# google-research/simclr

Measured on AMD Instinct MI355X. Metric: images/sec (whole node), ResNet-50 1x SimCLR pretraining step @224px, higher is better.
Workload: dtype f32; 1 GPU; ResNet-50 1x, 224x224, 2 views/image, per-GPU batch 512, global batch 512, NT-Xent T=0.1 + linear-eval head + LARS, global BN, dp1; global_batch=512, parallelism=dp1

## Files before the change

### simclr_amd/csrc/conv.hip

```cpp
#include "common.h"
#include <stdlib.h>
#include <string.h>
#include <mutex>
#include <type_traits>

namespace {

enum { MODE_FWD = 0, MODE_DGRAD = 1 };

struct ConvP {
  const void* x;
  const void* w;
  void* y;
  float* stats;
  int V, IH, IW, IC, OH, OW, N, KH, KW, stride, pad;
  int pixpitch;
  int M, K;
  int nslot, accumulate;
  int m_tiles, n_tiles;
  int cs, py, px, cls_h, cls_w;
  int ntaps;
  int taps[9];
  unsigned long long tap_w, dy_w, dx_w;
  const void* bn_x;
// ... 2158 lines not shown
      const int row = q >> 3, j = (q >> 2) & 1, gq = q & 3;
      u32x4* w0 = (u32x4*)(xs + off_of(row, (j * 8 + gq) * 16));
      u32x4* w1 = (u32x4*)(xs + off_of(row, (j * 8 + 4 + gq) * 16));
      u32x4 hi, lo;
      split_terms2(*w0, *w1, hi, lo);
      *w0 = hi; *w1 = lo;
    }
  };

  auto compute = [&](int s) __attribute__((always_inline)) {
    const unsigned char* xs = smem + s * stage_bytes;
    const unsigned char* ds = xs + p.hpp * RB;
    u32x4 dh[4], dl[4];
#pragma unroll
    for (int ni = 0; ni < 4; ++ni) {
      const int o0 = b_lo[ni] & ~7, o1 = hi_of(b_lo[ni]);
      dh[ni] = frag(ds, o0, o1);
      dl[ni] = frag(ds, o0 ^ 64, o1 ^ 64);
    }
    const int jw = p.W - gx;
    const unsigned lowm = jw >= 8 ? 0xffu : ((1u << jw) - 1u);
    const int y1 = (gy + 1 == p.H) ? 0 : gy + 1;
    const unsigned up = (gy > 0 ? lowm : 0u) | (y1 > 0 ? (0xffu & ~lowm) : 0u);
    const unsigned dn = (gy < p.H - 1 ? lowm : 0u) | (y1 < p.H - 1 ? (0xffu & ~lowm) : 0u);
    const unsigned lf = 0xffu & ~((gx == 0 ? 1u : 0u) | (jw < 8 ? (1u << jw) : 0u));
    const unsigned rt = 0xffu & ~((jw - 1 < 8 ? (1u << (jw - 1)) : 0u) | (jw - 1 + p.W < 8 ? (1u << (jw - 1 + p.W)) : 0u));
    __builtin_amdgcn_s_setprio(1);
#pragma unroll
    for (int t = 0; t < 9; ++t) {
      const int ty = t / 3, tx = t % 3;
      const int o0 = a_lo[t] & ~7, o1 = hi_of(a_lo[t]);
      u32x4 xh = frag(xs, o0, o1);
      u32x4 xl = frag(xs, o0 ^ 64, o1 ^ 64);
      if (t != 4) {
        const unsigned m8 = (ty == 0 ? up : ty == 2 ? dn : 0xffu) & (tx == 0 ? lf : tx == 2 ? rt : 0xffu);
#pragma unroll
        for (int d = 0; d < 4; ++d) {
          const unsigned w = ((unsigned)__builtin_amdgcn_sbfe((int)m8, 2 * d, 1) & 0x0000ffffu) |
                             ((unsigned)__builtin_amdgcn_sbfe((int)m8, 2 * d + 1, 1) & 0xffff0000u);
          xh[d] &= w; xl[d] &= w;
        }
      }
#pragma unroll
      for (int ni = 0; ni < 4; ++ni) acc[t][ni] = mma_bf16(dl[ni], xh, acc[t][ni]);
#pragma unroll
      for (int ni = 0; ni < 4; ++ni) acc[t][ni] = mma_bf16(dh[ni], xl, acc[t][ni]);
#pragma unroll
      for (int ni = 0; ni < 4; ++ni) acc[t][ni] = mma_bf16(dh[ni], xh, acc[t][ni]);
      __builtin_amdgcn_sched_barrier(0);
    }
    __builtin_amdgcn_s_setprio(0);
    gx += dcol;
    if (gx >= p.W) { gx -= p.W; ++gy; }
    gy += drow;
    if (gy >= p.H) gy -= p.H;
  };

  int issued = c_begin, cs = 0, is = 1;
  if (issued < c_end) { issue(issued, 0); ++issued; }
  for (int c = c_begin; c < c_end; ++c) {
    asm volatile("s_waitcnt vmcnt(0)" ::: "memory");
    __syncthreads();
    if (issued < c_end) { issue(issued, is); ++issued; is ^= 1; }
    convert(cs);
    __syncthreads();
    compute(cs);
    cs ^= 1;
  }
  float* slab = p.dw + (long long)split * 9 * p.IC * p.N;
  const int Qx = 4 * (wave & 1) + (fl >> 2);
  const int ci = ci0 + (wave >> 1) * 32 + (Qx & 1) * 16 + (Qx >> 1) * 4 + (fl & 3);
#pragma unroll
  for (int t = 0; t < 9; ++t) {
    const int kk = t * p.IC + ci;
#pragma unroll
    for (int ni = 0; ni < 4; ++ni) {
      const int Q = 4 * (ni & 1) + g;
      const int n = n0 + (ni >> 1) * 32 + (Q & 1) * 16 + (Q >> 1) * 4;
      *(float4*)(slab + (long long)kk * p.N + n) = make_float4(acc[t][ni][0], acc[t][ni][1], acc[t][ni][2], acc[t][ni][3]);
    }
  }
}

template <int TT>
__global__ __launch_bounds__(256) void small_gemm_nt_f32(const float* __restrict__ A, const float* __restrict__ B,
                                                         float* __restrict__ C, int M, int N, int K) {
  constexpr int LDR = 36;
  constexpr int FR = TT / 32;
  constexpr int LPT = TT * 8 / 256;
  __shared__ __attribute__((aligned(16))) float As[TT * LDR], Bs[TT * LDR];
  const int tid = threadIdx.x, lane = tid & 63, wave = tid >> 6;
  const int fl = lane & 15, q = lane >> 4;
  const int wm = wave >> 1, wn = wave & 1;
  const int m0 = blockIdx.y * TT, n0 = blockIdx.x * TT;
  f32x4 acc[FR][FR];
#pragma unroll
  for (int i = 0; i < FR; ++i)
#pragma unroll
    for (int j = 0; j < FR; ++j) acc[i][j] = (f32x4){0.f, 0.f, 0.f, 0.f};
  float4 ra[LPT], rb[LPT];
  auto gload = [&](int k0) __attribute__((always_inline)) {
#pragma unroll
    for (int l = 0; l < LPT; ++l) {
      const int idx = tid + l * 256, r = idx >> 3, c = (idx & 7) * 4;
      ra[l] = (m0 + r < M) ? *(const float4*)(A + (long long)(m0 + r) * K + k0 + c) : make_float4(0.f, 0.f, 0.f, 0.f);
      rb[l] = (n0 + r < N) ? *(const float4*)(B + (long long)(n0 + r) * K + k0 + c) : make_float4(0.f, 0.f, 0.f, 0.f);
    }
  };
  gload(0);
  for (int k0 = 0; k0 < K; k0 += 32) {
    __syncthreads();
#pragma unroll
    for (int l = 0; l < LPT; ++l) {
      const int idx = tid + l * 256, r = idx >> 3, c = (idx & 7) * 4;
      *(float4*)(As + r * LDR + c) = ra[l];
      *(float4*)(Bs + r * LDR + c) = rb[l];
    }
    __syncthreads();
    if (k0 + 32 < K) gload(k0 + 32);
#pragma unroll
    for (int h = 0; h < 2; ++h) {
      float4 af[FR], bf[FR];
#pragma unroll
      for (int i = 0; i < FR; ++i) {
        af[i] = *(const float4*)(As + (wm * (FR * 16) + i * 16 + fl) * LDR + h * 16 + 4 * q);
        bf[i] = *(const float4*)(Bs + (wn * (FR * 16) + i * 16 + fl) * LDR + h * 16 + 4 * q);
      }
#pragma unroll
      for (int i = 0; i < FR; ++i)
#pragma unroll
        for (int j = 0; j < FR; ++j) {
          acc[i][j] = __builtin_amdgcn_mfma_f32_16x16x4f32(bf[j].x, af[i].x, acc[i][j], 0, 0, 0);
          acc[i][j] = __builtin_amdgcn_mfma_f32_16x16x4f32(bf[j].y, af[i].y, acc[i][j], 0, 0, 0);
          acc[i][j] = __builtin_amdgcn_mfma_f32_16x16x4f32(bf[j].z, af[i].z, acc[i][j], 0, 0, 0);
          acc[i][j] = __builtin_amdgcn_mfma_f32_16x16x4f32(bf[j].w, af[i].w, acc[i][j], 0, 0, 0);
        }
    }
  }
#pragma unroll
  for (int i = 0; i < FR; ++i) {
    const int m = m0 + wm * (FR * 16) + i * 16 + fl;
#pragma unroll
    for (int j = 0; j < FR; ++j) {
      const int n = n0 + wn * (FR * 16) + j * 16 + q * 4;
      if (m < M && n < N) *(float4*)(C + (long long)m * N + n) = make_float4(acc[i][j][0], acc[i][j][1], acc[i][j][2], acc[i][j][3]);
    }
  }
}

__global__ __launch_bounds__(256) void slab_reduce(const float* __restrict__ slabs, int splits, long long numel,
                                                   float* __restrict__ out, int accumulate) {
  __shared__ float4 red[16][16];
  const long long n4 = numel / 4;
  const int tx = threadIdx.x & 15, sl = threadIdx.x >> 4;
  const long long i = blockIdx.x * 16ll + tx;
  float4 a = make_float4(0.f, 0.f, 0.f, 0.f);
  if (i < n4) {
    const float* src = slabs + i * 4;
    int s = sl;
    for (; s + 48 < splits; s += 64) {
      float4 v[4];
#pragma unroll
      for (int j = 0; j < 4; ++j) v[j] = *(const float4*)(src + (long long)(s + 16 * j) * numel);
#pragma unroll
      for (int j = 0; j < 4; ++j) { a.x += v[j].x; a.y += v[j].y; a.z += v[j].z; a.w += v[j].w; }
    }
// ... 584 lines not shown
static void run_igemm(dim3 grid, dim3 block, size_t lds, hipStream_t stream, const ConvP& p) {
  char name[128];
  snprintf(name, sizeof(name), "conv_igemm<%s, %s, %d, %s, %s>", type_name<T>(), mode_name(MODE), BN, tf(STATS), tf(GLDS));
  record_inst<T, MODE>(name, grid.x, block.x, lds, p);
  if (!dry_run()) hipLaunchKernelGGL((conv_igemm<T, MODE, BN, STATS, GLDS>), grid, block, lds, stream, p);
}

template <int MODE, bool STATS, bool BNEPI, bool FLAT>
static void run_wide(dim3 grid, dim3 block, size_t lds, hipStream_t stream, const ConvP& p) {
  char name[128];
  snprintf(name, sizeof(name), "conv_igemm_wide<%s, %s, %s, %s>", mode_name(MODE), tf(STATS), tf(BNEPI), tf(FLAT));
  record_inst<uint16_t, MODE>(name, grid.x, block.x, lds, p);
  if (!dry_run()) hipLaunchKernelGGL((conv_igemm_wide<MODE, STATS, BNEPI, FLAT>), grid, block, lds, stream, p);
}

template <typename T, int MODE, int BM, int BN, int NW, int STAGES, bool STATS, bool BNEPI, bool EXT = false,
          bool WIN = false, bool FAPPLY = false, int SPL = 0, bool TAIL = false, bool PSB = false, int FAS = 0, int EPS = 0, bool PSX = false>
static void run_persistent(dim3 grid, dim3 block, size_t lds, hipStream_t stream, const ConvP& p) {
  const int opt[9] = {EXT, WIN, FAPPLY, SPL, TAIL, PSB, FAS, EPS, PSX};
  const bool is_bool[9] = {true, true, true, false, true, true, false, false, true};
  int n = 9;
  while (n > 0 && opt[n - 1] == 0) --n;
  char name[256];
  int len = snprintf(name, sizeof(name), "conv_igemm_persistent<%s, %s, %d, %d, %d, %d, %s, %s", type_name<T>(), mode_name(MODE), BM, BN, NW,
                     STAGES, tf(STATS), tf(BNEPI));
  for (int i = 0; i < n; ++i)
    len += is_bool[i] ? snprintf(name + len, sizeof(name) - len, ", %s", tf(opt[i])) : snprintf(name + len, sizeof(name) - len, ", %d", opt[i]);
  snprintf(name + len, sizeof(name) - len, ">");
  record_inst<T, MODE>(name, grid.x, block.x, lds, p);
  if (!dry_run())
    hipLaunchKernelGGL((conv_igemm_persistent<T, MODE, BM, BN, NW, STAGES, STATS, BNEPI, EXT, WIN, FAPPLY, SPL, TAIL, PSB, FAS, EPS, PSX>),
                       grid, block, lds, stream, p);
}

template <int KPT, int FAS>
static void run_nwalk(dim3 grid, dim3 block, size_t lds, hipStream_t stream, const ConvP& p) {
  char name[64];
  snprintf(name, sizeof(name), "conv_igemm_nwalk<%d, %d>", KPT, FAS);
  record_inst<float, MODE_FWD>(name, grid.x, block.x, lds, p);
  const size_t len = strlen(g_last_inst);
  snprintf(g_last_inst + len, sizeof(g_last_inst) - len, " walk=n_inner n_group=%d n_groups=%d", p.nw_gw, p.nw_groups);
  if (!dry_run()) hipLaunchKernelGGL((conv_igemm_nwalk<KPT, FAS>), grid, block, lds, stream, p);
}

struct WgradRec { int k_tiles, n_tiles, splits, chunks_per_split, xcd_map; };
static WgradRec rec_of(const WgradP& p) { return {p.k_tiles, p.n_tiles, p.splits, p.chunks_per_split, p.xcd_map}; }
static WgradRec rec_of(const Wgrad3P& p) { return {p.ci_tiles, p.co_tiles, p.splits, p.chunks_per_split, 1}; }
static WgradRec rec_of(const StemWgP& p) { return {1, 1, p.splits, p.chunks_per_split, 0}; }
static void record_wgrad(const char* kern, int elt, const char* role, unsigned grid, unsigned block, size_t lds, const WgradRec& r) {
  snprintf(g_last_inst, sizeof(g_last_inst), "(%s) elt=%d role=%s grid=%u block=%u lds=%zu k_tiles=%d n_tiles=%d splits=%d chunks_per_split=%d xcd_map=%d",
           kern, elt, role, grid, block, lds, r.k_tiles, r.n_tiles, r.splits, r.chunks_per_split, r.xcd_map);
}

template <typename T, int BKW, int BNW, bool MT = false>
static void run_wgrad(const char* role, unsigned grid, unsigned block, size_t lds, hipStream_t stream, const WgradP& p) {
  char name[128];
  snprintf(name, sizeof(name), MT ? "conv_wgrad<%s, %d, %d, true>" : "conv_wgrad<%s, %d, %d>", type_name<T>(), BKW, BNW);
  record_wgrad(name, (int)sizeof(T), role, grid, block, lds, rec_of(p));
  if (!dry_run()) hipLaunchKernelGGL((conv_wgrad<T, BKW, BNW, MT>), dim3(grid), dim3(block), lds, stream, p);
}

template <typename T, int BKW, int BNW, int BRM, int STAGES, int WK = 2, int WNN = 2, bool GRAM = false, bool MT = false, int SPL = 0, int PSD = 0>
static void run_wgrad_dma(const char* role, unsigned grid, unsigned block, size_t lds, hipStream_t stream, const WgradP& p) {
  const int opt[6] = {WK, WNN, GRAM, MT, SPL, PSD}, dflt[6] = {2, 2, 0, 0, 0, 0};
  const bool is_bool[6] = {false, false, true, true, false, false};
  int n = 6;
  while (n > 0 && opt[n - 1] == dflt[n - 1]) --n;
  char name[160];
  int len = snprintf(name, sizeof(name), "conv_wgrad_dma<%s, %d, %d, %d, %d", type_name<T>(), BKW, BNW, BRM, STAGES);
  for (int i = 0; i < n; ++i)
    len += is_bool[i] ? snprintf(name + len, sizeof(name) - len, ", %s", tf(opt[i])) : snprintf(name + len, sizeof(name) - len, ", %d", opt[i]);
  snprintf(name + len, sizeof(name) - len, ">");
  record_wgrad(name, (int)sizeof(T), role, grid, block, lds, rec_of(p));
  if (!dry_run())
    hipLaunchKernelGGL((conv_wgrad_dma<T, BKW, BNW, BRM, STAGES, WK, WNN, GRAM, MT, SPL, PSD>), dim3(grid), dim3(block), lds, stream, p);
}

template <int ST> static void run_wgrad3x3_bf16(unsigned grid, unsigned block, size_t lds, hipStream_t stream, const Wgrad3P& q) {
  char name[64];
  snprintf(name, sizeof(name), "conv_wgrad3x3_bf16<%d>", ST);
  record_wgrad(name, 2, "wgrad", grid, block, lds, rec_of(q));
  if (!dry_run()) hipLaunchKernelGGL(conv_wgrad3x3_bf16<ST>, dim3(grid), dim3(block), lds, stream, q);
}
static void run_wgrad3x3_f32ps(unsigned grid, unsigned block, size_t lds, hipStream_t stream, const Wgrad3P& q) {
  record_wgrad("conv_wgrad3x3_f32ps", 4, "wgrad", grid, block, lds, rec_of(q));
  if (!dry_run()) hipLaunchKernelGGL(conv_wgrad3x3_f32ps, dim3(grid), dim3(block), lds, stream, q);
}
template <int STAGES> static void run_stem_wgrad_ps(unsigned grid, unsigned block, size_t lds, hipStream_t stream, const StemWgP& p) {
  char name[64];
  snprintf(name, sizeof(name), "stem_wgrad_ps<7, 2, %d>", STAGES);
  record_wgrad(name, 4, "stem_wgrad_ps", grid, block, lds, rec_of(p));
  if (!dry_run()) hipLaunchKernelGGL((stem_wgrad_ps<7, 2, STAGES>), dim3(grid), dim3(block), lds, stream, p);
}
static void run_slab_reduce(const void* slabs, int splits, long long numel, float* out, int accumulate, hipStream_t stream) {
  const int grid = max(1, (int)ceil_div(numel / 4, 16));
  const size_t len = strlen(g_last_inst);
  snprintf(g_last_inst + len, sizeof(g_last_inst) - len, " reduce_grid=%d", grid);
  if (!dry_run()) hipLaunchKernelGGL(slab_reduce, dim3(grid), dim3(256), 0, stream, (const float*)slabs, splits, numel, out, accumulate);
}

static const void* zero_page() {
  static void* zp = nullptr;
  if (dry_run()) return (const void*)&g_last_inst;
  if (!zp && hipGetSymbolAddress(&zp, HIP_SYMBOL(g_zero16)) != hipSuccess) zp = nullptr;
  return zp;
}

static void igemm_persistent_grid(long long M, int N, int* bn, int* n_tiles, int* grid, bool narrow = false) {
  const int BN = (N <= 64 || narrow) ? 64 : 128;
  const int m_tiles = (int)((M + 127) / 128);
  const int nt = ceil_div(N, BN);
  const int unit = 8 * nt;
  const int resident = (BN == 64 ? 3 : 2) * 256;
  int pg = (resident / unit) * unit;
  if (pg < unit) pg = unit;
  const int need = ceil_div(m_tiles, 8) * unit;
  if (pg > need) pg = need;
  *bn = BN; *n_tiles = nt; *grid = pg;
}

static bool igemm_use_256(const ConvP& p, bool fwd) {
  if (p.N % 256 != 0 || p.ntaps <= 0 || p.N / 256 > 32) return false;
  const char* e = getenv("SIMCLR_IGEMM_TILE");
  const int mode = e ? atoi(e) : 0;
  if (mode == 256) return true;
  if (mode == 128) return false;
  if (p.KH != 1 || p.KW != 1 || p.M < 150000) return false;
  if (p.bn_mode && !p.fapply) return false;
  if (fwd && !p.fapply && p.stats && p.K < 128) return false;
  return !p.fapply;
}

static bool f32_epi_batch() {
  const char* e = getenv("SIMCLR_F32_EPI_BATCH");
  return !e || atoi(e) != 0;
}

static constexpr bool f32_eps_exists(bool win, int eps) { return !win && (eps == 1 || eps == 4); }

static bool igemm_use_wide(const ConvP& p, bool fwd) {
  const char* e = getenv("SIMCLR_IGEMM_WIDE");
  const int mode = e ? atoi(e) : 1;
  if (mode == 0) return false;
  if (p.N % 256 != 0 || p.N / 256 > 32 || p.ntaps <= 0 || p.IC % 64 != 0 || p.x2 || p.fapply) return false;
  if (p.bn_mode && p.bn_mode != 4 && !p.bn_x) return false;
  if ((long long)p.V * p.IH * p.IW * p.pixpitch * 2 >= 0xE0000000ll || (long long)p.N * p.K * 2 >= 0xE0000000ll) return false;
  if (mode == 2) return true;
  if (p.M < 32768) return false;
  if (fwd) return !(p.KH == 3 && p.KW == 3 && p.stride == 1) && 2.0 * (double)p.M * p.K * p.N >= 3.0e11;
  return !p.bn_mode && !p.accumulate && p.KH == 1 && p.KW == 1 && p.IC >= 512;
}

static bool igemm_narrow(const ConvP& p, size_t esz, bool dgrad = false) {
  constexpr int kmax = 64;
  constexpr int kmax32 = 128;
  if (esz == 4)
    return dgrad && p.split == 3 && p.N > 64 && p.KH == 1 && p.KW == 1 && p.stride == 1 && !p.x2 && p.K <= kmax32 && p.N / 64 <= 64;
  return esz == 2 && p.N > 64 && p.KH == 1 && p.KW == 1 && p.stride == 1 && !p.x2 && p.K <= kmax && p.N / 64 <= 64;
}

static std::mutex g_scratch_mutex;

struct SplitScratch { hipStream_t stream; float* ws; size_t floats; unsigned* flags; size_t nflags; };
static SplitScratch g_split_scratch[8];
static int g_split_scratch_n = 0;

static thread_local int g_last_split_parts = 0;
static void split_tail_plan(ConvP& p, int grid, int units, int unit_steps, bool wide = false) {
  p.rem_parts = 0; p.rem_full = 0; p.rem_tiles = 0; p.part_ws = nullptr; p.part_flags = nullptr; p.part_err = nullptr;
// ... 413 lines not shown
          }
      q.M = p.V * q.cls_h * q.cls_w;
      if (q.ntaps == 0 && p.accumulate == 2 && ((py | px) & 1)) q.accumulate = 0;
      else if (q.ntaps == 0 && p.accumulate) continue;
      if (p.accumulate == 3) q.accumulate = 0;
      if (q.ntaps == 0) q.x_ps = 0;
      if (plan_igemm<T, MODE>(q, true, true).family == IgemmPlan::UNSUPPORTED) return 1;
      cls[n++] = q;
    }
  for (int i = 0; i < n; ++i)
    if (int rc = launch_igemm_one<T, MODE>(cls[i], stream)) return rc;
  return 0;
}

struct ConvCall { int dtype, terms; bool w_ps, x_ps; };
static int conv_call(const char* fn, int dtype, bool fwd, int ps_w_terms, bool ps_in, int Cout, ConvCall* c) {
  c->terms = terms_of(&dtype, fwd);
  SIMCLR_CHECK_ARG(c->terms >= 0, "%s: bad matrix-arithmetic field in dtype (SIMCLR_FMT_TERMS)", fn);
  c->w_ps = ps_w_terms && take_ps_w(&dtype);
  SIMCLR_CHECK_ARG(!c->w_ps || ((dtype & 0xff) == SIMCLR_DT_F32 && c->terms == ps_w_terms),
                   "%s: pre-split weights (SIMCLR_FMT_PS_W) need fp32 storage and terms %d", fn, ps_w_terms);
  c->x_ps = ps_in && (dtype & SIMCLR_FMT_PS_IN) != 0;
  if (ps_in) dtype &= 0xff;
  SIMCLR_CHECK_ARG(!c->x_ps || (dtype == SIMCLR_DT_F32 && c->terms == 3 && Cout % 32 == 0),
                   "%s: a pre-split dy needs fp32 storage, three backward terms (simclr_set_f32_matmul) and Cout %% 32 == 0", fn);
  c->dtype = dtype;
  return 0;
}
static int conv_params(const ConvCall& c, const void* x, const void* w, void* y, int V, int IH, int IW, int IC, int OH, int OW, int N,
                       int KH, int KW, int stride, int pad, ConvP* p) {
  *p = {};
  p->zero = zero_page();
  SIMCLR_CHECK_ARG(p->zero != nullptr, "conv2d: zero page symbol not found");
  p->w_ps = c.w_ps ? 1 : 0; p->x_ps = c.x_ps ? 1 : 0;
  p->split = c.terms;
  p->x = x; p->w = w; p->y = y;
  p->V = V; p->IH = IH; p->IW = IW; p->IC = IC; p->OH = OH; p->OW = OW; p->N = N;
  p->KH = KH; p->KW = KW; p->stride = stride; p->pad = pad; p->pixpitch = IC;
  p->M = V * OH * OW; p->K = KH * KW * IC;
  return 0;
}
template <int MODE> static int launch_conv(int dtype, const ConvP& p, hipStream_t stream) {
  return dtype == SIMCLR_DT_BF16 ? launch_igemm<uint16_t, MODE>(p, stream) : launch_igemm<float, MODE>(p, stream);
}


static int env_int(const char* name, int dflt) { const char* e = getenv(name); return e ? atoi(e) : dflt; }

static int wgrad_splits(long long M, int K, int N, int bkw, int bnw, int br, int* chunks_per_split, int cap, int target) {
  const int tiles = ceil_div(K, bkw) * ceil_div(N, bnw);
  const int nchunks = ceil_div(M, br);
  int splits = max(1, min(nchunks, target / max(1, tiles)));
  if (nchunks >= 8) splits = min(nchunks / 8 * 8, max(8, (splits + 7) / 8 * 8));
  splits = min(splits, cap);
  *chunks_per_split = ceil_div(nchunks, splits);
  int eff = ceil_div(nchunks, *chunks_per_split);
  while (nchunks >= 8 && eff % 8 != 0 && *chunks_per_split > 1) {
    --*chunks_per_split;
    eff = ceil_div(nchunks, *chunks_per_split);
    if (eff > cap) { ++*chunks_per_split; eff = ceil_div(nchunks, *chunks_per_split); break; }
  }
  return eff;
}

struct WgradShape { int V, IH, IW, Cin, pixpitch, OH, OW, Cout, KH, KW, stride, pad; };
struct WgradPlan {
  enum Family {
    UNSUPPORTED,
    NINE_TAP_BF16,
    NINE_TAP_F32PS,
    TILE256_BF16,
    TILE256_F32,
    STEM_DMA_BF16,
    STEM_DMA_F32,
    STEM_MT,
    REG_STAGED,
    DMA_RING,
    GRAM,
    STEM_PS
  } family;
  int bkw, bnw;
  int stages, br;
  int hpp;
  int splits, chunks_per_split;
  int k_tiles, n_tiles, xcd_map;
  unsigned grid, block;
  size_t lds;
};

static bool wgrad_takes_presplit(const WgradShape& s, int dtype, int terms) {
  return dtype == SIMCLR_DT_F32 && terms == 3 && s.Cin % 64 == 0 && s.Cout % 32 == 0 && (s.pixpitch * 4) % 16 == 0;
}

static WgradPlan plan_wgrad(const WgradShape& s, int dtype, int terms, bool dy_ps) {
  WgradPlan k = {};
  const bool bf = dtype == SIMCLR_DT_BF16;
  const int esz = bf ? 2 : 4, taps = s.KH * s.KW, K = taps * s.Cin, N = s.Cout;
  const long long M = (long long)s.V * s.OH * s.OW;
  const bool aligned = (s.pixpitch * esz) % 16 == 0;
  k.block = 256;
  if (env_int("SIMCLR_WGRAD_3X3", 1) > 0 && s.KH == 3 && s.KW == 3 && s.stride == 1 && s.pad == 1 && s.IH == s.OH && s.IW == s.OW &&
      s.Cin % 64 == 0 && s.Cout % 64 == 0 && s.IW >= 7 && (bf ? aligned : (terms == 3 && dy_ps))) {
    const int br = bf ? 64 : 32;
    const int hpp = (br + 2 * s.IW + 2 + 31) / 32 * 32;
    const size_t stage = (size_t)(hpp + br) * 64 * esz;
    if ((bf ? 2 : 4) * stage <= 160 * 1024) {
      k.family = bf ? WgradPlan::NINE_TAP_BF16 : WgradPlan::NINE_TAP_F32PS;
      k.bkw = 64; k.bnw = 64; k.br = br; k.hpp = hpp;
      k.stages = (bf && 2 * 3 * stage <= 160 * 1024) ? 3 : 2;
      k.k_tiles = s.Cin / 64; k.n_tiles = N / 64;
      const int tiles = k.k_tiles * k.n_tiles;
      const int want = min(bf ? 4096 : 2048, max(8, env_int("SIMCLR_WGRAD3_BLOCKS", tiles == 1 ? 2048 : 512)));
      k.splits = wgrad_splits(M, s.Cin, N, 64, 64, br, &k.chunks_per_split, 2048, want);
      k.xcd_map = 1;
      k.grid = tiles * ceil_div(k.splits, 8) * 8;
      k.lds = k.stages * stage;
      return k;
    }
  }
  k.bkw = (s.Cin % 128 == 0) ? 128 : (s.Cin % 64 == 0 ? 64 : 32);
  k.bnw = (N % 128 == 0 || N > 128) ? 128 : 64;
  if (k.bkw == 32) k.bnw = 64;
  if (s.Cin % 256 == 0 && N % 256 == 0 && aligned) {
    if (bf && env_int("SIMCLR_WGRAD_256", 1) != 0 && (M >= 500000 || (taps == 9 && M >= 150000 && s.Cin == 256))) k.bkw = k.bnw = 256;
    if (!bf && terms == 3 && dy_ps && s.stride == 1 && taps == 1) k.bkw = k.bnw = 256;
  }
  const bool stem = k.bkw == 32 && s.Cin == 32 && K <= 256 && N <= 64;
  if (stem) { k.bkw = 256; k.bnw = 64; }
  int cfg = env_int("SIMCLR_WGRAD_CFG", -1);
  if (cfg < 0 || (!bf && cfg > 1)) cfg = 1;
  if (k.bkw == 32 || stem || !aligned) cfg = 0;
  const bool big = k.bkw == 128 && k.bnw == 128, big256 = k.bkw == 256 && !stem;
  if (big256 && cfg == 0) cfg = 1;
  if (dy_ps && cfg == 0) return k;
  const int brm = ((cfg >= 2 && big) || (big256 && bf)) ? 1 : 2;
  k.stages = big256 ? (bf ? 4 : 2) : (cfg <= 1 ? 2 : (big ? (cfg == 2 ? 3 : 4) : 3));
  k.br = (bf ? 32 : 16) * brm;
  const int target = stem ? 1024 : (k.bkw == 256 ? 512 : env_int("SIMCLR_WGRAD_BLOCKS", bf ? 1024 : 1536));
  k.splits = wgrad_splits(M, K, N, k.bkw, k.bnw, k.br, &k.chunks_per_split, stem ? 1024 : 256, target);
  k.k_tiles = ceil_div(K, k.bkw);
  k.n_tiles = ceil_div(N, k.bnw);
  k.xcd_map = cfg != 0 || M >= 1500000 || (M >= 500000 && taps == 1 && s.stride == 1);
#ifdef SIMCLR_DIAG
  { const char* e = getenv("SIMCLR_WGRAD_XCD"); if (e && atoi(e) >= 0) k.xcd_map = atoi(e); }
#endif
  k.family = big256 ? (bf ? WgradPlan::TILE256_BF16 : WgradPlan::TILE256_F32) : cfg == 0 ? WgradPlan::REG_STAGED : WgradPlan::DMA_RING;
  if (big256) k.block = 512;
  if (stem) {
    const bool packed = s.KW == 1 && s.pad == 0 && s.pixpitch == 4;
    k.family = WgradPlan::STEM_MT;
    if (bf && packed && s.stride % 2 == 0 && s.IW % 2 == 0) {
      k.family = WgradPlan::STEM_DMA_BF16;
    } else if (!bf && packed && terms != 0 && env_int("SIMCLR_STEM_SPLIT", 1) != 0) {
      k.family = WgradPlan::STEM_DMA_F32;
      k.block = 512;
      if (terms == 3 && env_int("SIMCLR_STEM_WGRAD_STAGES", 2) == 3) k.stages = 3;
    }
    if (k.family != WgradPlan::STEM_MT) k.xcd_map = 1;
  }
  k.grid = k.k_tiles * k.n_tiles * (k.xcd_map ? ceil_div(k.splits, 8) * 8 : k.splits);
  k.lds = (size_t)k.stages * k.br * (k.bkw + k.bnw) * esz;
  return k;
}

static WgradPlan plan_gram(long long M, int K, int dtype) {
  WgradPlan k = {};
  const bool bf = dtype == SIMCLR_DT_BF16;
  k.family = WgradPlan::GRAM;
  k.bkw = k.bnw = K;
  k.stages = 4;
  k.br = (bf ? 64 : 32) / (K == 256 ? 2 : 1);
  const int ranges = K == 256 ? 512 : 1024;
  k.splits = wgrad_splits(M, K, K, K, K, k.br, &k.chunks_per_split, ranges, ranges);
  k.k_tiles = 1; k.n_tiles = 1; k.xcd_map = 1;
  k.grid = ceil_div(k.splits, 8) * 8;
  k.block = K == 256 ? 512 : 256;
  k.lds = (size_t)k.stages * k.br * K * (bf ? 2 : 4);
  return k;
}

static WgradPlan plan_stem_wgrad_ps(int V, int OH, int OW) {
  WgradPlan k = {};
  k.family = WgradPlan::STEM_PS;
  k.bkw = 7 * 32; k.bnw = 64; k.br = 32;
  const long long chunks = (long long)V * OH * ((OW + 31) / 32);
  const int want = (int)max(1ll, min((long long)max(8, min(env_int("SIMCLR_STEM_WGRAD_BLOCKS", 1024), 1024)), chunks));
  k.chunks_per_split = (int)((chunks + want - 1) / want);
  k.splits = (int)((chunks + k.chunks_per_split - 1) / k.chunks_per_split);
  k.stages = env_int("SIMCLR_STEM_WGRAD_PS_STAGES", 2) == 3 ? 3 : 2;
  k.k_tiles = 1; k.n_tiles = 1;
  k.grid = k.splits; k.block = 128;
  k.lds = (size_t)k.stages * ((7 * 70 + 63) / 64 + 8) * 1024;
  return k;
}

template <int A, int B> struct WgradTile { static constexpr int BKW = A, BNW = B; };
template <typename F> static void with_wgrad_tile(int bkw, int bnw, F&& f) {
  if (bkw == 128 && bnw == 128) f(WgradTile<128, 128>());
  else if (bkw == 128) f(WgradTile<128, 64>());
// ... 207 lines not shown
  ConvCall c;
  if (int rc = conv_call("conv2d_dgrad_bn_ext", dtype, false, 0, false, Cout, &c)) return rc;
  dtype = c.dtype;
  const int epc = dtype == SIMCLR_DT_BF16 ? 8 : 4;
  SIMCLR_CHECK_ARG(dtype == SIMCLR_DT_BF16 || dtype == SIMCLR_DT_F32, "conv2d_dgrad_bn_ext: bad dtype %d", dtype);
  SIMCLR_CHECK_ARG(Cout % (8 * epc) == 0 && Cin % (8 * epc) == 0, "conv2d_dgrad_bn_ext: Cin=%d / Cout=%d must be multiples of %d", Cin, Cout, 8 * epc);
  SIMCLR_CHECK_ARG((long long)V * H * W < (1ll << 31), "conv2d_dgrad_bn_ext: M overflows int32");
  SIMCLR_CHECK_ARG(mask_mode >= 1 && mask_mode <= 4, "conv2d_dgrad_bn_ext: mask_mode must be 1, 2, 3 or 4");
  SIMCLR_CHECK_ARG(dm && h && w_ext && stats && nslot > 0 && (mask_mode == 4 || (bn_x && bn_mean && bn_rstd)), "conv2d_dgrad_bn_ext: null argument");
  SIMCLR_CHECK_ARG(mask_mode == 2 || bn_mask, "conv2d_dgrad_bn_ext: mask_mode 1 / 3 / 4 need bn_mask");
  SIMCLR_CHECK_ARG(mask_mode != 2 || (bn_scale && bn_shift), "conv2d_dgrad_bn_ext: mask_mode 2 needs scale/shift");
  ConvP p;
  if (int rc = conv_params(c, dm, w_ext, dx, V, H, W, Cout, H, W, Cin, 1, 1, 1, 0, &p)) return rc;
  p.stats = stats; p.nslot = nslot; p.accumulate = accumulate;
  p.K = Cout + Cin;
  p.x2 = h; p.ic2 = Cin; p.pixpitch2 = Cin; p.bias = bias;
  p.bn_x = bn_x; p.bn_mask = bn_mask; p.bn_scale = bn_scale; p.bn_shift = bn_shift;
  p.bn_mean = bn_mean; p.bn_rstd = bn_rstd; p.bn_mode = mask_mode;
  SIMCLR_CHECK_ARG(launch_conv<MODE_DGRAD>(dtype, p, stream) == 0, "conv2d_dgrad_bn_ext: no kernel for this launch");
  SIMCLR_CHECK_LAUNCH();
  return 0;
}

int simclr_conv2d_dgrad_ext(const void* dm, const void* h, const void* w_ext, const float* bias, void* dx, int accumulate,
                            int V, int H, int W, int Cin, int Cout, int dtype, hipStream_t stream) {
  ConvCall c;
  if (int rc = conv_call("conv2d_dgrad_ext", dtype, false, 0, false, Cout, &c)) return rc;
  dtype = c.dtype;
  const int epc = dtype == SIMCLR_DT_BF16 ? 8 : 4;
  SIMCLR_CHECK_ARG(dtype == SIMCLR_DT_BF16 || dtype == SIMCLR_DT_F32, "conv2d_dgrad_ext: bad dtype %d", dtype);
  SIMCLR_CHECK_ARG(Cout % (8 * epc) == 0 && Cin % (8 * epc) == 0, "conv2d_dgrad_ext: Cin=%d / Cout=%d must be multiples of %d", Cin, Cout, 8 * epc);
  SIMCLR_CHECK_ARG((long long)V * H * W < (1ll << 31), "conv2d_dgrad_ext: M overflows int32");
  SIMCLR_CHECK_ARG(dm && h && w_ext && dx, "conv2d_dgrad_ext: null argument");
  ConvP p;
  if (int rc = conv_params(c, dm, w_ext, dx, V, H, W, Cout, H, W, Cin, 1, 1, 1, 0, &p)) return rc;
  p.nslot = 1; p.accumulate = accumulate;
  p.K = Cout + Cin;
  p.x2 = h; p.ic2 = Cin; p.pixpitch2 = Cin; p.bias = bias;
  SIMCLR_CHECK_ARG(launch_conv<MODE_DGRAD>(dtype, p, stream) == 0, "conv2d_dgrad_ext: no kernel for this launch");
  SIMCLR_CHECK_LAUNCH();
  return 0;
}

size_t simclr_conv2d_wgrad_workspace_bytes(int V, int OH, int OW, int Cin, int Cout, int KH, int KW, int dtype) {
  int splits = 0;
  for (int stride = 1; stride <= 2; ++stride)
    for (int odd_pitch = 0; odd_pitch <= 1; ++odd_pitch) {
      const WgradShape s = {V, OH * stride, OW * stride, Cin, Cin + odd_pitch, OH, OW, Cout, KH, KW, stride, (KH - 1) / 2};
      for (int terms : {0, 3, 6})
        for (int ps = 0; ps <= 1; ++ps) {
          if (dtype == SIMCLR_DT_BF16 ? (terms != 0 || ps) : (!valid_terms(terms, false) || (ps && !wgrad_takes_presplit(s, dtype, terms)))) continue;
          const WgradPlan k = plan_wgrad(s, dtype, terms, ps != 0);
          if (k.family != WgradPlan::UNSUPPORTED) splits = max(splits, k.splits);
        }
    }
  return (size_t)splits * KH * KW * Cin * Cout * sizeof(float);
}

int simclr_conv2d_wgrad(const void* x, const void* dy, float* dw, int accumulate, void* workspace,
                        int V, int IH, int IW, int Cin, int pixpitch, int OH, int OW, int Cout, int KH,
                        int KW, int stride, int pad, int dtype, hipStream_t stream) {
  const int terms = terms_of(&dtype, false);
  SIMCLR_CHECK_ARG(terms >= 0, "conv2d_wgrad: bad matrix-arithmetic field in dtype (SIMCLR_FMT_TERMS)");
  const bool dy_ps = (dtype & SIMCLR_FMT_PS_IN) != 0;
  dtype &= 0xff;
  const WgradShape s = {V, IH, IW, Cin, pixpitch, OH, OW, Cout, KH, KW, stride, pad};
  SIMCLR_CHECK_ARG(!dy_ps || wgrad_takes_presplit(s, dtype, terms),
                   "conv2d_wgrad: a pre-split dy needs fp32 storage, three backward terms, Cin %% 64 == 0 and Cout %% 32 == 0 (Cin=%d Cout=%d)", Cin, Cout);
  SIMCLR_CHECK_ARG(dtype == SIMCLR_DT_BF16 || dtype == SIMCLR_DT_F32, "conv2d_wgrad: bad dtype %d", dtype);
  SIMCLR_CHECK_ARG(Cin % 32 == 0, "conv2d_wgrad: Cin=%d must be a multiple of 32", Cin);
  SIMCLR_CHECK_ARG(Cout % 8 == 0, "conv2d_wgrad: Cout=%d must be a multiple of 8", Cout);
  SIMCLR_CHECK_ARG((long long)V * OH * OW < (1ll << 31), "conv2d_wgrad: M overflows int32");
  const WgradPlan k = plan_wgrad(s, dtype, terms, dy_ps);
  SIMCLR_CHECK_ARG(k.family != WgradPlan::UNSUPPORTED, "conv2d_wgrad: no pre-split kernel on the register-staged path");
  const void* zero = zero_page();
  SIMCLR_CHECK_ARG(zero != nullptr, "conv2d_wgrad: zero page symbol not found");
  const int M = V * OH * OW, K = KH * KW * Cin;
  if (k.family == WgradPlan::NINE_TAP_BF16 || k.family == WgradPlan::NINE_TAP_F32PS) {
    Wgrad3P q = {};
    q.x = x; q.dy = dy; q.dw = (float*)workspace; q.zero = zero;
    q.V = V; q.H = IH; q.W = IW; q.IC = Cin; q.N = Cout; q.pixpitch = pixpitch; q.M = M;
    q.ci_tiles = k.k_tiles; q.co_tiles = k.n_tiles;
    q.splits = k.splits; q.chunks_per_split = k.chunks_per_split; q.hpp = k.hpp;
    if (k.family == WgradPlan::NINE_TAP_F32PS) run_wgrad3x3_f32ps(k.grid, k.block, k.lds, stream, q);
    else if (k.stages == 3) run_wgrad3x3_bf16<3>(k.grid, k.block, k.lds, stream, q);
    else run_wgrad3x3_bf16<2>(k.grid, k.block, k.lds, stream, q);
  } else {
    WgradP p = {};
    p.x = x; p.dy = dy; p.dw = (float*)workspace; p.zero = zero;
    p.V = V; p.IH = IH; p.IW = IW; p.IC = Cin; p.OH = OH; p.OW = OW; p.N = Cout;
    p.KH = KH; p.KW = KW; p.stride = stride; p.pad = pad; p.pixpitch = pixpitch;
    p.M = M; p.K = K;
    p.splits = k.splits; p.chunks_per_split = k.chunks_per_split;
    p.k_tiles = k.k_tiles; p.n_tiles = k.n_tiles; p.xcd_map = k.xcd_map;
    p.split = terms;
    p.dy_ps = dy_ps ? 1 : 0;
#ifdef SIMCLR_DIAG
    { const char* e = getenv("SIMCLR_DIAG"); p.diag = e ? atoi(e) : 0; }
#endif
    launch_wgrad(k, dtype == SIMCLR_DT_BF16, stream, p);
  }
  SIMCLR_CHECK_LAUNCH();
  run_slab_reduce(workspace, k.splits, (long long)K * Cout, dw, accumulate, stream);
  SIMCLR_CHECK_LAUNCH();
  return 0;
}

size_t simclr_conv2d_gram_workspace_bytes(long long M, int K, int dtype) {
  return (size_t)plan_gram(M, K, dtype).splits * ((size_t)K * K + K) * sizeof(float);
}
int simclr_conv2d_gram(const void* h, float* out, void* workspace, long long M, int K, int dtype, hipStream_t stream) {
  const int terms = terms_of(&dtype, true);
  SIMCLR_CHECK_ARG(terms >= 0, "conv2d_gram: bad matrix-arithmetic field in dtype (SIMCLR_FMT_TERMS)");
  SIMCLR_CHECK_ARG(dtype == SIMCLR_DT_BF16 || dtype == SIMCLR_DT_F32, "conv2d_gram: bad dtype %d", dtype);
  SIMCLR_CHECK_ARG(K == 64 || K == 128 || (K == 256 && dtype == SIMCLR_DT_BF16), "conv2d_gram: K=%d not supported (64, 128, bf16 256)", K);
  SIMCLR_CHECK_ARG(M > 0 && M < (1ll << 31), "conv2d_gram: bad M");
  const WgradPlan k = plan_gram(M, K, dtype);
  WgradP p = {};
  p.x = h; p.dy = h; p.dw = (float*)workspace;
  p.V = 1; p.IH = 1; p.IW = (int)M; p.IC = K; p.OH = 1; p.OW = (int)M; p.N = K;
  p.KH = 1; p.KW = 1; p.stride = 1; p.pad = 0; p.pixpitch = K;
  p.M = (int)M; p.K = K;
  p.splits = k.splits; p.chunks_per_split = k.chunks_per_split;
  p.k_tiles = k.k_tiles; p.n_tiles = k.n_tiles; p.xcd_map = k.xcd_map;
  p.zero = zero_page();
  SIMCLR_CHECK_ARG(p.zero != nullptr, "conv2d_gram: zero page symbol not found");
  if (K == 256) run_wgrad_dma<uint16_t, 256, 256, 1, 4, 2, 4, true>("gram", k.grid, k.block, k.lds, stream, p);
  else if (dtype == SIMCLR_DT_BF16) {
    if (K == 64) run_wgrad_dma<uint16_t, 64, 64, 2, 4, 2, 2, true>("gram", k.grid, k.block, k.lds, stream, p);
    else run_wgrad_dma<uint16_t, 128, 128, 2, 4, 2, 2, true>("gram", k.grid, k.block, k.lds, stream, p);
  } else if (terms != 0) {
    if (K == 64) run_wgrad_dma<float, 64, 64, 2, 4, 2, 2, true, false, 6>("gram", k.grid, k.block, k.lds, stream, p);
    else run_wgrad_dma<float, 128, 128, 2, 4, 2, 2, true, false, 6>("gram", k.grid, k.block, k.lds, stream, p);
  } else {
    if (K == 64) run_wgrad_dma<float, 64, 64, 2, 4, 2, 2, true>("gram", k.grid, k.block, k.lds, stream, p);
    else run_wgrad_dma<float, 128, 128, 2, 4, 2, 2, true>("gram", k.grid, k.block, k.lds, stream, p);
  }
  SIMCLR_CHECK_LAUNCH();
  run_slab_reduce(workspace, k.splits, (long long)K * K + K, out, 0, stream);
  SIMCLR_CHECK_LAUNCH();
  return 0;
}

int simclr_small_gemm_nt_f32(const float* A, const float* B, float* C, int M, int N, int K, hipStream_t stream) {
  SIMCLR_CHECK_ARG(M > 0 && N > 0 && K > 0 && M % 16 == 0 && N % 16 == 0 && K % 32 == 0, "small_gemm_nt_f32: M=%d N=%d must be multiples of 16, K=%d of 32", M, N, K);
  if ((long long)ceil_div(M, 64) * ceil_div(N, 64) >= 256)
    hipLaunchKernelGGL((small_gemm_nt_f32<64>), dim3(ceil_div(N, 64), ceil_div(M, 64)), dim3(256), 0, stream, A, B, C, M, N, K);
  else
    hipLaunchKernelGGL((small_gemm_nt_f32<32>), dim3(ceil_div(N, 32), ceil_div(M, 32)), dim3(256), 0, stream, A, B, C, M, N, K);
  SIMCLR_CHECK_LAUNCH();
  return 0;
}

int simclr_stem_conv_fwd(const void* xp, const void* w_s, void* y, float* stats, int nslot, int V,
                         int HP, int WP, int OH, int OW, int Cout, int KHP, int KWP, int stride,
                         int dtype, hipStream_t stream) {
  const int terms = terms_of(&dtype, true);
  SIMCLR_CHECK_ARG(terms >= 0, "stem_conv_fwd: bad matrix-arithmetic field in dtype (SIMCLR_FMT_TERMS)");
  SIMCLR_CHECK_ARG(dtype == SIMCLR_DT_BF16 || dtype == SIMCLR_DT_F32, "stem_conv_fwd: bad dtype %d", dtype);
  const int epc = dtype == SIMCLR_DT_BF16 ? 8 : 4;
  StemP p = {};
  p.xp = xp; p.w = w_s; p.y = y; p.stats = stats; p.nslot = nslot > 0 ? nslot : 1;
  p.V = V; p.HP = HP; p.WP = WP; p.OH = OH; p.OW = OW; p.N = Cout; p.KHP = KHP; p.KWP = KWP;
  p.stride = stride; p.M = V * OH * OW; p.KP = KHP * KWP * 4;
  SIMCLR_CHECK_ARG(p.KP % (4 * epc) == 0, "stem_conv_fwd: padded K=%d not a multiple of %d", p.KP, 4 * epc);
  SIMCLR_CHECK_ARG((KWP * 4) % epc == 0, "stem_conv_fwd: KWP*4 must be a multiple of %d", epc);
  SIMCLR_CHECK_ARG(Cout % (dtype == SIMCLR_DT_BF16 ? 8 : 4) == 0, "stem_conv_fwd: Cout=%d must be a multiple of %d", Cout, dtype == SIMCLR_DT_BF16 ? 8 : 4);
// ... 137 lines not shown
```

Measured before the change: 3729 images/s.

## Add rolling-ring LDS variant of fp32 pre-split 3x3 wgrad kernel

Adds a 3x3 weight-gradient kernel for fp32 pre-split inputs that keeps the input halo in a circular LDS ring of 128 or 256 rows. Each chunk loads and bf16-splits only the BR new rows instead of reloading the whole halo window, so global traffic and conversion work fall. The smaller LDS footprint also allows two blocks per CU, and shapes whose halo was too large for the old kernel can now take this path. Wide feature maps get fewer split blocks by default, and the planner picks the ring size.

```diff
diff --git a/simclr_amd/csrc/conv.hip b/simclr_amd/csrc/conv.hip
--- a/simclr_amd/csrc/conv.hip
+++ b/simclr_amd/csrc/conv.hip
@@ -2264,6 +2264,178 @@
   }
 }
 
+template <int R>
+__global__ __launch_bounds__(256, 2) void conv_wgrad3x3_f32ps_roll(const Wgrad3P p) {
+  constexpr int BR = 32, RB = 256;
+  constexpr int RMASK = R * RB - 1;
+  extern __shared__ __attribute__((aligned(16))) unsigned char smem[];
+  typedef __attribute__((address_space(1))) const void* gptr_t;
+  typedef __attribute__((address_space(3))) void* lptr_t;
+  const int tid = threadIdx.x, lane = tid & 63;
+  const int wave = __builtin_amdgcn_readfirstlane(tid >> 6);
+  const int g = lane >> 4, fl = lane & 15;
+  const int tiles = p.ci_tiles * p.co_tiles;
+  const int xcd = blockIdx.x & 7, bidx = blockIdx.x >> 3;
+  const int tile = bidx % tiles, split = (bidx / tiles) * 8 + xcd;
+  if (split >= p.splits) return;
+  const int ci0 = (tile % p.ci_tiles) * 64, n0 = (tile / p.ci_tiles) * 64;
+  const float* __restrict__ X = (const float*)p.x;
+  const float* __restrict__ DY = (const float*)p.dy;
+  const int W1 = p.W + 1;
+  unsigned char* const gs = smem + R * RB;
+
+  f32x4 acc[9][4];
+#pragma unroll
+  for (int t = 0; t < 9; ++t)
+#pragma unroll
+    for (int j = 0; j < 4; ++j) acc[t][j] = (f32x4){0.f, 0.f, 0.f, 0.f};
+
+  const int nchunks = (p.M + BR - 1) / BR;
+  const int c_begin = split * p.chunks_per_split;
+  const int c_end = min(nchunks, c_begin + p.chunks_per_split);
+
+  const int lrow = lane >> 4, lpc = lane & 15;
+  auto issue_x = [&](int v0, int nrows) __attribute__((always_inline)) {
+    const int nxi = nrows >> 2;
+    for (int q = wave; q < nxi; q += 4) {
+      const int v = v0 + q * 4 + lrow;
+      const int lc = (((lpc >> 1) ^ w3f_key(v)) << 1) | (lpc & 1);
+      const int gp = v - W1;
+      const void* src = (gp >= 0 && gp < p.M) ? (const void*)(X + (long long)gp * p.pixpitch + ci0 + lc * 4) : p.zero;
+      __builtin_amdgcn_global_load_lds((gptr_t)src, (lptr_t)(smem + (((v0 + q * 4) & (R - 1)) * RB)), 16, 0, 0);
+    }
+  };
+  auto issue_dy = [&](int c, int s) __attribute__((always_inline)) {
+    unsigned char* ds = gs + s * (BR * RB);
+    const int mc = c * BR;
+#pragma unroll
+    for (int j = 0; j < 2; ++j) {
+      const int q = wave * 2 + j;
+      const int r = q * 4 + lrow;
+      const int lc = (((lpc >> 1) ^ w3f_key(r)) << 1) | (lpc & 1);
+      const int m = mc + r;
+      const void* src = (m < p.M) ? (const void*)(DY + (long long)m * p.N + n0 + lc * 4) : p.zero;
+      __builtin_amdgcn_global_load_lds((gptr_t)src, (lptr_t)(ds + q * 1024), 16, 0, 0);
+    }
+  };
+
+  auto off_of = [&](int row, int byte) -> int { return row * RB + (((byte >> 5) ^ w3f_key(row)) << 5) + (byte & 31); };
+  const int px_lane = g * 8 + (fl >> 2);
+  const int xbyte = (wave >> 1) * 128 + (wave & 1) * 32 + (fl & 3) * 8;
+  auto hi_of = [](int o) __attribute__((always_inline)) -> int { return ((o & ~7) + 4 * RB) ^ ((o & 1) << 7); };
+  int a_lo[9];
+#pragma unroll
+  for (int t = 0; t < 9; ++t) {
+    const int r = px_lane + W1 + (t / 3 - 1) * p.W + (t % 3 - 1);
+    a_lo[t] = off_of((c_begin * BR + r) & (R - 1), xbyte) | ((r >> 2) & 1);
+  }
+  int b_lo[4];
+#pragma unroll
+  for (int ni = 0; ni < 4; ++ni) {
+    const int nbyte = (ni >> 1) * 128 + (ni & 1) * 32 + (fl & 3) * 8;
+    b_lo[ni] = off_of(px_lane, nbyte) | ((px_lane >> 2) & 1);
+  }
+  auto frag = [&](const unsigned char* base, int o_lo, int o_hi) __attribute__((always_inline)) -> u32x4 {
+    const s16x4_t lo = __builtin_amdgcn_ds_read_tr16_b64_v4i16((lds_s16x4_t*)(base + o_lo));
+    const s16x4_t hi = __builtin_amdgcn_ds_read_tr16_b64_v4i16((lds_s16x4_t*)(base + o_hi));
+    const u32x2 l2 = __builtin_bit_cast(u32x2, lo), h2 = __builtin_bit_cast(u32x2, hi);
+    return (u32x4){l2[0], l2[1], h2[0], h2[1]};
+  };
+
+  const int hw = p.H * p.W;
+  const int dq = BR / hw, drem = BR - dq * hw, drow = drem / p.W, dcol = drem - drow * p.W;
+  int gy, gx;
+  {
+    const int m = c_begin * BR + g * 8;
+    const int rem = m % hw;
+    gy = rem / p.W; gx = rem - gy * p.W;
+  }
+
+  auto convert = [&](int v0, int nrows) __attribute__((always_inline)) {
+    for (int q = tid; q < nrows * 8; q += 256) {
+      const int row = (v0 + (q >> 3)) & (R - 1), j = (q >> 2) & 1, gq = q & 3;
+      u32x4* w0 = (u32x4*)(smem + off_of(row, (j * 8 + gq) * 16));
+      u32x4* w1 = (u32x4*)(smem + off_of(row, (j * 8 + 4 + gq) * 16));
+      u32x4 hi, lo;
+      split_terms2(*w0, *w1, hi, lo);
+      *w0 = hi; *w1 = lo;
+    }
+  };
+
+  auto compute = [&](int s) __attribute__((always_inline)) {
+    const unsigned char* ds = gs + s * (BR * RB);
+    u32x4 dh[4], dl[4];
+#pragma unroll
+    for (int ni = 0; ni < 4; ++ni) {
+      const int o0 = b_lo[ni] & ~7, o1 = hi_of(b_lo[ni]);
+      dh[ni] = frag(ds, o0, o1);
+      dl[ni] = frag(ds, o0 ^ 64, o1 ^ 64);
+    }
+    const int jw = p.W - gx;
+    const unsigned lowm = jw >= 8 ? 0xffu : ((1u << jw) - 1u);
+    const int y1 = (gy + 1 == p.H) ? 0 : gy + 1;
+    const unsigned up = (gy > 0 ? lowm : 0u) | (y1 > 0 ? (0xffu & ~lowm) : 0u);
+    const unsigned dn = (gy < p.H - 1 ? lowm : 0u) | (y1 < p.H - 1 ? (0xffu & ~lowm) : 0u);
+    const unsigned lf = 0xffu & ~((gx == 0 ? 1u : 0u) | (jw < 8 ? (1u << jw) : 0u));
+    const unsigned rt = 0xffu & ~((jw - 1 < 8 ? (1u << (jw - 1)) : 0u) | (jw - 1 + p.W < 8 ? (1u << (jw - 1 + p.W)) : 0u));
+    __builtin_amdgcn_s_setprio(1);
+#pragma unroll
+    for (int t = 0; t < 9; ++t) {
+      const int ty = t / 3, tx = t % 3;
+      const int o0 = a_lo[t] & ~7, o1 = hi_of(a_lo[t]) & RMASK;
+      u32x4 xh = frag(smem, o0, o1);
+      u32x4 xl = frag(smem, o0 ^ 64, o1 ^ 64);
+      a_lo[t] = (a_lo[t] + BR * RB) & RMASK;
+      if (t != 4) {
+        const unsigned m8 = (ty == 0 ? up : ty == 2 ? dn : 0xffu) & (tx == 0 ? lf : tx == 2 ? rt : 0xffu);
+#pragma unroll
+        for (int d = 0; d < 4; ++d) {
+          const unsigned w = ((unsigned)__builtin_amdgcn_sbfe((int)m8, 2 * d, 1) & 0x0000ffffu) |
+                             ((unsigned)__builtin_amdgcn_sbfe((int)m8, 2 * d + 1, 1) & 0xffff0000u);
+          xh[d] &= w; xl[d] &= w;
+        }
+      }
+#pragma unroll
+      for (int ni = 0; ni < 4; ++ni) acc[t][ni] = mma_bf16(dl[ni], xh, acc[t][ni]);
+#pragma unroll
+      for (int ni = 0; ni < 4; ++ni) acc[t][ni] = mma_bf16(dh[ni], xl, acc[t][ni]);
+#pragma unroll
+      for (int ni = 0; ni < 4; ++ni) acc[t][ni] = mma_bf16(dh[ni], xh, acc[t][ni]);
+      __builtin_amdgcn_sched_barrier(0);
+    }
+    __builtin_amdgcn_s_setprio(0);
+    gx += dcol;
+    if (gx >= p.W) { gx -= p.W; ++gy; }
+    gy += drow;
+    if (gy >= p.H) gy -= p.H;
+  };
+
+  if (c_begin < c_end) { issue_x(c_begin * BR, p.hpp); issue_dy(c_begin, 0); }
+  int cs = 0;
+  for (int c = c_begin; c < c_end; ++c) {
+    asm volatile("s_waitcnt vmcnt(0)" ::: "memory");
+    __syncthreads();
+    if (c + 1 < c_end) { issue_x(c * BR + p.hpp, BR); issue_dy(c + 1, cs ^ 1); }
+    if (c == c_begin) convert(c * BR, p.hpp); else convert(c * BR + p.hpp - BR, BR);
+    __syncthreads();
+    compute(cs);
+    cs ^= 1;
+  }
+  float* slab = p.dw + (long long)split * 9 * p.IC * p.N;
+  const int Qx = 4 * (wave & 1) + (fl >> 2);
+  const int ci = ci0 + (wave >> 1) * 32 + (Qx & 1) * 16 + (Qx >> 1) * 4 + (fl & 3);
+#pragma unroll
+  for (int t = 0; t < 9; ++t) {
+    const int kk = t * p.IC + ci;
+#pragma unroll
+    for (int ni = 0; ni < 4; ++ni) {
+      const int Q = 4 * (ni & 1) + g;
+      const int n = n0 + (ni >> 1) * 32 + (Q & 1) * 16 + (Q >> 1) * 4;
+      *(float4*)(slab + (long long)kk * p.N + n) = make_float4(acc[t][ni][0], acc[t][ni][1], acc[t][ni][2], acc[t][ni][3]);
+    }
+  }
+}
+
 template <int TT>
 __global__ __launch_bounds__(256) void small_gemm_nt_f32(const float* __restrict__ A, const float* __restrict__ B,
                                                          float* __restrict__ C, int M, int N, int K) {
@@ -3014,9 +3186,14 @@
   record_wgrad(name, 2, "wgrad", grid, block, lds, rec_of(q));
   if (!dry_run()) hipLaunchKernelGGL(conv_wgrad3x3_bf16<ST>, dim3(grid), dim3(block), lds, stream, q);
 }
-static void run_wgrad3x3_f32ps(unsigned grid, unsigned block, size_t lds, hipStream_t stream, const Wgrad3P& q) {
+static void run_wgrad3x3_f32ps(int ring, unsigned grid, unsigned block, size_t lds, hipStream_t stream, const Wgrad3P& q) {
   record_wgrad("conv_wgrad3x3_f32ps", 4, "wgrad", grid, block, lds, rec_of(q));
-  if (!dry_run()) hipLaunchKernelGGL(conv_wgrad3x3_f32ps, dim3(grid), dim3(block), lds, stream, q);
+  const size_t len = strlen(g_last_inst);
+  snprintf(g_last_inst + len, sizeof(g_last_inst) - len, ring ? " roll=1 ring=%d" : " roll=0", ring);
+  if (dry_run()) return;
+  if (ring == 0) hipLaunchKernelGGL(conv_wgrad3x3_f32ps, dim3(grid), dim3(block), lds, stream, q);
+  else if (ring == 128) hipLaunchKernelGGL(conv_wgrad3x3_f32ps_roll<128>, dim3(grid), dim3(block), lds, stream, q);
+  else hipLaunchKernelGGL(conv_wgrad3x3_f32ps_roll<256>, dim3(grid), dim3(block), lds, stream, q);
 }
 template <int STAGES> static void run_stem_wgrad_ps(unsigned grid, unsigned block, size_t lds, hipStream_t stream, const StemWgP& p) {
   char name[64];
@@ -3596,6 +3773,7 @@
   int bkw, bnw;
   int stages, br;
   int hpp;
+  int ring;
   int splits, chunks_per_split;
   int k_tiles, n_tiles, xcd_map;
   unsigned grid, block;
@@ -3618,17 +3796,21 @@
     const int br = bf ? 64 : 32;
     const int hpp = (br + 2 * s.IW + 2 + 31) / 32 * 32;
     const size_t stage = (size_t)(hpp + br) * 64 * esz;
-    if ((bf ? 2 : 4) * stage <= 160 * 1024) {
+    const int roll = bf ? 0 : env_int("SIMCLR_WGRAD3_ROLL", 1);
+    const int ring = (roll != 0 && hpp + 32 <= 256 && (roll >= 2 || s.IW <= 47)) ? (hpp + 32 <= 128 ? 128 : 256) : 0;
+    if (ring != 0 || (bf ? 2 : 4) * stage <= 160 * 1024) {
       k.family = bf ? WgradPlan::NINE_TAP_BF16 : WgradPlan::NINE_TAP_F32PS;
       k.bkw = 64; k.bnw = 64; k.br = br; k.hpp = hpp;
       k.stages = (bf && 2 * 3 * stage <= 160 * 1024) ? 3 : 2;
       k.k_tiles = s.Cin / 64; k.n_tiles = N / 64;
       const int tiles = k.k_tiles * k.n_tiles;
-      const int want = min(bf ? 4096 : 2048, max(8, env_int("SIMCLR_WGRAD3_BLOCKS", tiles == 1 ? 2048 : 512)));
+      const bool wide_ring = ring != 0 && s.IW >= 48;
+      const int want = min(bf ? 4096 : 2048, max(8, env_int("SIMCLR_WGRAD3_BLOCKS", (tiles == 1 && !wide_ring) ? 2048 : 512)));
       k.splits = wgrad_splits(M, s.Cin, N, 64, 64, br, &k.chunks_per_split, 2048, want);
       k.xcd_map = 1;
       k.grid = tiles * ceil_div(k.splits, 8) * 8;
-      k.lds = k.stages * stage;
+      k.ring = ring;
+      k.lds = ring ? (size_t)(ring + 2 * br) * 64 * esz : k.stages * stage;
       return k;
     }
   }
@@ -4002,7 +4184,7 @@
     q.V = V; q.H = IH; q.W = IW; q.IC = Cin; q.N = Cout; q.pixpitch = pixpitch; q.M = M;
     q.ci_tiles = k.k_tiles; q.co_tiles = k.n_tiles;
     q.splits = k.splits; q.chunks_per_split = k.chunks_per_split; q.hpp = k.hpp;
-    if (k.family == WgradPlan::NINE_TAP_F32PS) run_wgrad3x3_f32ps(k.grid, k.block, k.lds, stream, q);
+    if (k.family == WgradPlan::NINE_TAP_F32PS) run_wgrad3x3_f32ps(k.ring, k.grid, k.block, k.lds, stream, q);
     else if (k.stages == 3) run_wgrad3x3_bf16<3>(k.grid, k.block, k.lds, stream, q);
     else run_wgrad3x3_bf16<2>(k.grid, k.block, k.lds, stream, q);
   } else {
```

Result: no change. 3748 images/s, median of 6 (+0.5%).
